# DethRaid/AndroidRenderer

Hardware: AMD Instinct MI355X
Metric: lit Mpixels/sec (deferred+GI pass) at 4K (higher is better)
Workload: dtype f32

## Files before the change

androidrenderer_amd/csrc/lighting.hip:

```cpp
#include <hip/hip_runtime.h>

#include <type_traits>

#include "../../include/sah_hip.h"
#include "fast_pixel_map.hpp"
#include "lighting_common.hpp"
#include "lighting_fast.hpp"
#include "launch.hpp"
#include "numerics.hpp"
#include "params.hpp"

namespace sah {

template <int SUN, int GI, int PPT>
__global__ void __launch_bounds__(256) k_lighting_general(const LightingArgs a, const CsmArgs csm, const LpvArgs lpv, const SkyArgs sky) {
    __shared__ float s_lut[512];
    stage_format_tables(s_lut, a.luts);
    __syncthreads();

    const uint32_t groups_per_row = a.width / PPT;
    const uint32_t gid = blockIdx.x * 256u + threadIdx.x;
    const uint32_t rows = a.row_end - a.row_begin;
    if (gid >= groups_per_row * rows) return;
    const uint32_t ry = gid / groups_per_row;
// ... 124 lines not shown
    bool neg_zero = false;
    auto put = [&](uint32_t at, float v) {
        out[at] = v;
        neg_zero = neg_zero || __float_as_uint(v) == 0x80000000u;
    };
    if (i < a.width) {
        put(i, colx_glsl_of(a, f, i));
        put(stride + i, colx_slang_of(a, f, i));
    }
    if (i < a.height) {
        put(2u * stride + i, rowy_glsl_of(a, f, i));
        put(2u * stride + row_stride + i, rowy_slang_of(a, f, i));
    }
    if (wave_any(neg_zero) && (threadIdx.x & 63u) == 0u) atomicOr(&f.state->colx_neg_zero, 1u);
}


template <int SUN, int GI, int PPT, bool SKY>
__global__ void __launch_bounds__(256, SKY ? 4 : 1) k_lighting_fast(const LightingArgs a, const CsmArgs csm, const LpvArgs lpv, const SkyArgs sky,
                                                                                 const FastArgs f) {
    uint32_t block_id = blockIdx.x;
    if (SKY) {
        if (blockIdx.x < f.sky_first) {
            const uint32_t ratio = f.sky_ratio;
            const uint32_t groups_per_row = a.width / PPT, rows = a.row_end - a.row_begin, total = groups_per_row * rows;
#pragma unroll 1
            for (uint32_t k = 0; k < ratio; k++) {
                const uint32_t gid = (blockIdx.x * ratio + k) * 256u + threadIdx.x;
                if (gid >= total) break;
                const FastPixel at = fast_pixel_of(gid, groups_per_row, rows, PPT, f.tile_rows, f.row_magic);
                const uint32_t y = a.row_begin + at.row, x0 = at.x0;
                uint32_t wz[PPT];
                load_words<PPT>(a.depth.ptr + (size_t)y * a.depth.pitch + (size_t)x0 * 4, wz);
#pragma unroll 1
                for (int i = 0; i < PPT; i++) {
                    if (__uint_as_float(wz[i]) != 0.f) continue;
                    Hn lit[4];
                    sky_frag(a, sky, x0 + (uint32_t)i, y, lit);
                    *reinterpret_cast<uint2*>(const_cast<uint8_t*>(a.lit.ptr) + (size_t)y * a.lit.pitch + (size_t)(x0 + i) * 8) = pack_lit(lit);
                }
            }
            return;
        }
        block_id = blockIdx.x - f.sky_first;
    }
    const uint32_t groups_per_row = a.width / PPT;
    const uint32_t gid = block_id * 256u + threadIdx.x;
    const uint32_t rows = a.row_end - a.row_begin;
    const bool active = gid < groups_per_row * rows;
    FastPixel at = {0u, 0u};
    if (active) at = fast_pixel_of(gid, groups_per_row, rows, PPT, f.tile_rows, f.row_magic);
    const uint32_t y = a.row_begin + at.row;
    const uint32_t x0 = at.x0;
    const bool lpv_bad = (GI == SAH_GI_LPV) ? (f.state->nonfinite != 0u) : false;
    const bool div_shared = (SUN == SAH_SHADOW_MODE_CSM || GI == SAH_GI_LPV) ? pos_div_shared_of(f) : false;

    uint32_t wc[PPT], wd[PPT], we[PPT], wz[PPT], wn[2 * PPT], wao[PPT], wm[PPT];
    float colx_g[PPT], colx_s[PPT];
    if (active) {
        load_words<PPT>(a.color.ptr + (size_t)y * a.color.pitch + (size_t)x0 * 4, wc);
        load_words<PPT>(a.data.ptr + (size_t)y * a.data.pitch + (size_t)x0 * 4, wd);
        load_words<PPT>(a.emission.ptr + (size_t)y * a.emission.pitch + (size_t)x0 * 4, we);
        load_words<PPT>(a.depth.ptr + (size_t)y * a.depth.pitch + (size_t)x0 * 4, wz);
        load_words<2 * PPT>(a.normals.ptr + (size_t)y * a.normals.pitch + (size_t)x0 * 8, wn);
        if (GI == SAH_GI_LPV && a.has_ao) load_words<PPT>(a.ao.ptr + (size_t)y * a.ao.pitch + (size_t)x0 * 4, wao);
        if (SUN == SAH_SHADOW_MODE_RT && a.has_mask) load_words<PPT>(a.shadow_mask.ptr + (size_t)y * a.shadow_mask.pitch + (size_t)x0 * 4, wm);
        if (f.colx_tab) {
            uint32_t t[PPT];
            if (SUN == SAH_SHADOW_MODE_CSM || GI == SAH_GI_LPV) {
                load_words<PPT>(reinterpret_cast<const uint8_t*>(f.colx_tab + x0), t);
#pragma unroll
                for (int i = 0; i < PPT; i++) colx_g[i] = __uint_as_float(t[i]);
            }
            if (SUN == SAH_SHADOW_MODE_RT) {
                load_words<PPT>(reinterpret_cast<const uint8_t*>(f.colx_tab + f.colx_stride + x0), t);
#pragma unroll
                for (int i = 0; i < PPT; i++) colx_s[i] = __uint_as_float(t[i]);
            }
        }
    }
    __shared__ __attribute__((aligned(16))) float s_lut[TAB_SIZE];
    stage_fast_tables<SUN == SAH_SHADOW_MODE_CSM, GI == SAH_GI_LPV>(s_lut, a, csm, f);
    __syncthreads();

    float rowy_glsl = 0.f, rowy_slang = 0.f;
    if (f.colx_tab) {
        if (SUN == SAH_SHADOW_MODE_CSM || GI == SAH_GI_LPV) rowy_glsl = f.colx_tab[2u * f.colx_stride + y];
        if (SUN == SAH_SHADOW_MODE_RT) rowy_slang = f.colx_tab[2u * f.colx_stride + f.rowy_stride + y];
    } else {
        if (SUN == SAH_SHADOW_MODE_CSM || GI == SAH_GI_LPV) rowy_glsl = rowy_glsl_of(a, f, y);
        if (SUN == SAH_SHADOW_MODE_RT) rowy_slang = rowy_slang_of(a, f, y);
    }

    uint32_t out[2 * PPT];
    uint32_t deferred_mask = 0, sky_mask = 0;
    bool emissive_wave;
    {
        uint32_t any_e = 0;
#pragma unroll
        for (int i = 0; i < PPT; i++) any_e |= we[i];
        emissive_wave = wave_any(active && (any_e & 0xffffffu) != 0u);
    }
#pragma unroll
    for (int i = 0; i < PPT; i++) {
        if (!active) break;
        Px p;
        p.color = wc[i];
        p.data = wd[i];
        p.emission = we[i];
        p.n01 = wn[2 * i];
        p.n23 = wn[2 * i + 1];
        p.depth = __uint_as_float(wz[i]);
        p.ao = (GI == SAH_GI_LPV && a.has_ao) ? __uint_as_float(wao[i]) : 1.0f;
        p.mask = (SUN == SAH_SHADOW_MODE_RT && a.has_mask) ? __uint_as_float(wm[i]) : 1.0f;
        const uint32_t x = x0 + i;
        float colx_glsl = 0.f, colx_slang = 0.f;
        if (f.colx_tab) {
            if (SUN == SAH_SHADOW_MODE_CSM || GI == SAH_GI_LPV) colx_glsl = colx_g[i];
            if (SUN == SAH_SHADOW_MODE_RT) colx_slang = colx_s[i];
        } else {
            if (SUN == SAH_SHADOW_MODE_CSM || GI == SAH_GI_LPV) colx_glsl = colx_glsl_of(a, f, x);
            if (SUN == SAH_SHADOW_MODE_RT) colx_slang = colx_slang_of(a, f, x);
        }
        const FastPixelOut r = shade_pixel_fast_sl<SUN, GI>(a, csm, lpv, f, colx_glsl, rowy_glsl, colx_slang, rowy_slang, p, s_lut, lpv_bad, emissive_wave, div_shared);
        out[2 * i] = r.lit.x;
        out[2 * i + 1] = r.lit.y;
        if (r.deferred) deferred_mask |= 1u << i;
        if (p.depth == 0.f) sky_mask |= 1u << i;
    }
    if (active) {
        uint8_t* dst = const_cast<uint8_t*>(a.lit.ptr) + (size_t)y * a.lit.pitch + (size_t)x0 * 8;
        if (SKY && sky_mask != 0u) {
#pragma unroll
            for (int i = 0; i < PPT; i++)
                if (!((sky_mask >> i) & 1u)) *reinterpret_cast<uint2*>(dst + 8 * i) = make_uint2(out[2 * i], out[2 * i + 1]);
        } else if constexpr (PPT == 1) {
            *reinterpret_cast<uint2*>(dst) = make_uint2(out[0], out[1]);
        } else {
            store_words<2 * PPT>(dst, out);
        }
    }
    const uint32_t seg = gid >> 6, lane = threadIdx.x & 63u;
    uint32_t front = 0;
    const uint32_t listed = SKY ? deferred_mask & ~sky_mask : deferred_mask;
    if (wave_any(listed != 0u)) {
        uint8_t* seg_codes = f.seg_list + (size_t)seg * f.seg_stride;
#pragma unroll
        for (int i = 0; i < PPT; i++) {
            const bool mine = (listed >> i) & 1u;
            const uint64_t m = __ballot(mine);
            if (m) {
                const uint32_t before = __builtin_amdgcn_mbcnt_hi((uint32_t)(m >> 32), __builtin_amdgcn_mbcnt_lo((uint32_t)m, 0u));
                if (mine) seg_codes[front + before] = (uint8_t)(lane * PPT + (uint32_t)i);
                front += (uint32_t)__builtin_popcountll(m);
            }
        }
    }
    if (lane == 0 && seg < f.num_segments) {
        f.seg_count[seg] = (uint16_t)front;
        if (front != 0u) f.state->deferred_hint[f.hint_slot] = 1u;
    }
    if (gid == 0u) f.state->deferred_hint[f.hint_slot ^ 1u] = 0u;
}

static hipError_t launch_lpv_pack(const LpvArgs& lpv, const FastArgs& f, hipStream_t st) {
    const uint32_t prows = (lpv.red.height + 2 * kLpvPackBorder) * (lpv.red.depth + 2 * kLpvPackBorder);
    const hipError_t me = hipMemsetAsync(&f.state->nonfinite, 0, sizeof(uint32_t), st);
    if (me != hipSuccess) return me;
    hipLaunchKernelGGL(k_lpv_pack, dim3(prows), dim3(256), 0, st, lpv.red, lpv.green, lpv.blue, const_cast<uint8_t*>(f.lpv_packed), f.pk_row_pitch,
                       f.pk_slice_pitch, f.state);
    return hipGetLastError();
}
template <int SUN, int GI>
static hipError_t launch_general_ppt(const LightingArgs& a, const CsmArgs& csm, const LpvArgs& lpv, const SkyArgs& sky, int ppt, hipStream_t st) {
    const uint32_t rows = a.row_end - a.row_begin;
    const uint64_t groups = (uint64_t)(a.width / ppt) * rows;
    if (groups == 0) return hipSuccess;
    const dim3 grid((uint32_t)((groups + 255) / 256)), block(256);
    if (ppt == 4) hipLaunchKernelGGL((k_lighting_general<SUN, GI, 4>), grid, block, 0, st, a, csm, lpv, sky);
    else if (ppt == 2) hipLaunchKernelGGL((k_lighting_general<SUN, GI, 2>), grid, block, 0, st, a, csm, lpv, sky);
    else hipLaunchKernelGGL((k_lighting_general<SUN, GI, 1>), grid, block, 0, st, a, csm, lpv, sky);
    return hipGetLastError();
}

template <int SUN, int GI>
static hipError_t launch_fast_ppt(const LightingArgs& a, const CsmArgs& csm, const LpvArgs& lpv, const SkyArgs& sky, const FastArgs& f, int ppt,
                                  hipStream_t st) {
    const uint32_t rows = a.row_end - a.row_begin;
    const uint64_t groups = (uint64_t)(a.width / ppt) * rows;
    if (groups == 0) return hipSuccess;
    if (GI == SAH_GI_LPV && f.repack) {
        const hipError_t pe = launch_lpv_pack(lpv, f, st);
        if (pe != hipSuccess) return pe;
    }
    const uint32_t blocks = (uint32_t)((groups + 255) / 256);
    const dim3 block(256);
    auto launch = [&](auto ppt_c) {
        constexpr int P = decltype(ppt_c)::value;
        if (sky.enabled) hipLaunchKernelGGL((k_lighting_fast<SUN, GI, P, true>), dim3(f.sky_first + blocks), block, 0, st, a, csm, lpv, sky, f);
        else hipLaunchKernelGGL((k_lighting_fast<SUN, GI, P, false>), dim3(blocks), block, 0, st, a, csm, lpv, sky, f);
    };
    if (ppt == 4) launch(std::integral_constant<int, 4>{});
    else if (ppt == 2) launch(std::integral_constant<int, 2>{});
    else launch(std::integral_constant<int, 1>{});
    const uint32_t fgroups = (f.num_segments + kFixupSegs - 1) / kFixupSegs;
    const dim3 fgrid(fgroups < kFixupMaxWorkgroups ? fgroups : kFixupMaxWorkgroups);
    if (ppt == 4) hipLaunchKernelGGL((k_lighting_fixup<SUN, GI, 4>), fgrid, block, 0, st, a, csm, lpv, sky, f);
// ... 44 lines not shown
```

androidrenderer_amd/csrc/lighting_common.hpp:

```cpp
#pragma once
#include <hip/hip_runtime.h>

#include "../../include/sah_hip.h"
#include "numerics.hpp"
#include "params.hpp"

namespace sah {

template <int NW> SAH_DEV void load_words(const uint8_t* p, uint32_t (&w)[NW]) {
    if constexpr (NW == 1) {
        w[0] = *reinterpret_cast<const uint32_t*>(p);
    } else if constexpr (NW == 2) {
        uint2 v = *reinterpret_cast<const uint2*>(p);
        w[0] = v.x; w[1] = v.y;
    } else if constexpr (NW == 4) {
        uint4 v = *reinterpret_cast<const uint4*>(p);
        w[0] = v.x; w[1] = v.y; w[2] = v.z; w[3] = v.w;
    } else {
        static_assert(NW == 8, "unsupported width");
        uint4 v0 = *reinterpret_cast<const uint4*>(p);
        uint4 v1 = *reinterpret_cast<const uint4*>(p + 16);
        w[0] = v0.x; w[1] = v0.y; w[2] = v0.z; w[3] = v0.w;
        w[4] = v1.x; w[5] = v1.y; w[6] = v1.z; w[7] = v1.w;
    }
}
template <int NW> SAH_DEV void store_words(uint8_t* p, const uint32_t (&w)[NW]) {
    if constexpr (NW == 2) {
        *reinterpret_cast<uint2*>(p) = make_uint2(w[0], w[1]);
    } else if constexpr (NW == 4) {
        *reinterpret_cast<uint4*>(p) = make_uint4(w[0], w[1], w[2], w[3]);
    } else {
        static_assert(NW == 8, "unsupported width");
        *reinterpret_cast<uint4*>(p) = make_uint4(w[0], w[1], w[2], w[3]);
        *reinterpret_cast<uint4*>(p + 16) = make_uint4(w[4], w[5], w[6], w[7]);
    }
}

struct Px {
    uint32_t color, data, emission, n01, n23;
    float depth, ao, mask;
};

SAH_DEV int clamp_to_int(float f) { return (int)__builtin_fminf(__builtin_fmaxf(f, -1.0e9f), 1.0e9f); }
SAH_DEV int clamp_index(float f, int hi) {
    int i, r;
    asm("v_cvt_i32_f32 %0, %1" : "=v"(i) : "v"(f));
    asm("v_med3_i32 %0, %1, 0, %2" : "=v"(r) : "v"(i), "s"(hi));
    return r;
}
SAH_DEV _Float16 hbits(uint32_t b) { return __builtin_bit_cast(_Float16, (uint16_t)b); }


struct TriSetup {
    float w[8];
    int x0, y0, z0;
    bool nan;
};
SAH_DEV TriSetup tri_setup(uint32_t W, uint32_t H, uint32_t D, float u, float v, float ww) {
    TriSetup s;
    const float px = u * (float)W - 0.5f, py = v * (float)H - 0.5f, pz = ww * (float)D - 0.5f;
    s.nan = isnan_f(px) || isnan_f(py) || isnan_f(pz);
    const float fx0 = __builtin_floorf(px), fy0 = __builtin_floorf(py), fz0 = __builtin_floorf(pz);
    const float fx = px - fx0, fy = py - fy0, fz = pz - fz0;
    const float wx0 = 1.0f - fx, wy0 = 1.0f - fy, wz0 = 1.0f - fz;
    s.x0 = clamp_to_int(fx0);
    s.y0 = clamp_to_int(fy0);
    s.z0 = clamp_to_int(fz0);
    const float wxy[4] = {wx0 * wy0, fx * wy0, wx0 * fy, fx * fy};
#pragma unroll
    for (int k = 0; k < 8; k++) s.w[k] = wxy[k & 3] * ((k >> 2) ? fz : wz0);
    return s;
}
typedef _Float16 half4_t __attribute__((ext_vector_type(4)));

SAH_DEV half4_t load_texel8_border(const VolumeArg& v, int x, int y, int z) {
    if ((unsigned)x < v.width && (unsigned)y < v.height && (unsigned)z < v.depth) {
        const uint32_t off = (uint32_t)z * v.slice_pitch + (uint32_t)y * v.row_pitch + (uint32_t)x * 8u;
        return *reinterpret_cast<const half4_t*>(v.ptr + off);
    }
    return half4_t{(_Float16)0.f, (_Float16)0.f, (_Float16)0.f, (_Float16)0.f};
}
SAH_DEV void tri_accumulate(const VolumeArg& v, const TriSetup& s, float (&out)[4]) {
    if (s.nan) {
        out[0] = out[1] = out[2] = out[3] = __builtin_nanf("");
        return;
    }
    half4_t t[8];
#pragma unroll
    for (int k = 0; k < 8; k++) t[k] = load_texel8_border(v, s.x0 + (k & 1), s.y0 + ((k >> 1) & 1), s.z0 + (k >> 2));
    out[0] = out[1] = out[2] = out[3] = 0.0f;
// ... 159 lines not shown
    s.base_color = {Hn(si.color[0]), Hn(si.color[1]), Hn(si.color[2])};
    s.normal = normalize(H3{Hn(si.normal[0]), Hn(si.normal[1]), Hn(si.normal[2])});
    s.roughness = Hn(si.rough);
    s.metalness = Hn(si.metal);
    const F3 location = worldspace_location_slang(a, (float)x, (float)y, p.depth);
    const F3 L = {Fn(a.sun_L[0]), Fn(a.sun_L[1]), Fn(a.sun_L[2])};
    const Hn ndotl = Hn(nclamp(dot(L, to_f(s.normal)), Fn(0.f), Fn(1.f)).v);
    const H3 V = to_h(normalize(location - F3{Fn(a.view_pos[0]), Fn(a.view_pos[1]), Fn(a.view_pos[2])}));
    const H3 Lh = to_h(L);
    const H3 b = brdf_sl(s, Lh, V);
    const H3 nb = ndotl * b;
    F3 radiance = to_f(nb) * F3{Fn(a.sun_color[0]), Fn(a.sun_color[1]), Fn(a.sun_color[2])};
    if (tof(ndotl) > 0.f) radiance = radiance * Fn(p.mask);
    const Fn exposure = Fn(0.00031415927f);
    add[0] = (radiance.x * exposure).v;
    add[1] = (radiance.y * exposure).v;
    add[2] = (radiance.z * exposure).v;
}

SAH_DEV void dir_to_sh(F3 d, Fn (&o)[4]) {
    const Fn c0 = Fn(0.282094792f), c1 = Fn(0.488602512f);
    o[0] = c0;
    o[1] = -c1 * d.y;
    o[2] = c1 * d.z;
    o[3] = -c1 * d.x;
}
SAH_DEV Fn dot4(const float (&t)[4], const Fn (&n)[4]) { return Fn(t[0]) * n[0] + Fn(t[1]) * n[1] + Fn(t[2]) * n[2] + Fn(t[3]) * n[3]; }

SAH_DEV void lpv_fetch(const LpvArgs& L, F4 p, const Fn (&n)[4], Fn (&out)[3]) {
    const TriSetup s = tri_setup(L.red.width, L.red.height, L.red.depth, p.x.v, p.y.v, p.z.v);
    float r[4], g[4], b[4];
    tri_accumulate(L.red, s, r);
    tri_accumulate(L.green, s, g);
    tri_accumulate(L.blue, s, b);
    out[0] = dot4(r, n);
    out[1] = dot4(g, n);
    out[2] = dot4(b, n);
}

SAH_DEV void lpv_fetch_packed(const LpvArgs& L, const uint8_t* packed, uint32_t row_pitch, uint32_t slice_pitch, float u, float v, float w,
                              const Fn (&n)[4], Fn (&out)[3]) {
    const int W = (int)L.red.width, H = (int)L.red.height, D = (int)L.red.depth;
    const float px = u * (float)W - 0.5f, py = v * (float)H - 0.5f, pz = w * (float)D - 0.5f;
    const float fx0 = __builtin_floorf(px), fy0 = __builtin_floorf(py), fz0 = __builtin_floorf(pz);
    const float fx = px - fx0, fy = py - fy0, fz = pz - fz0;
    const float gx = 1.0f - fx, gy = 1.0f - fy, gz = 1.0f - fz;
    const int b = (int)kLpvPackBorder;
    const uint32_t x0 = (uint32_t)(min(max(clamp_to_int(fx0), -b), W) + b), y0 = (uint32_t)(min(max(clamp_to_int(fy0), -b), H) + b),
                   z0 = (uint32_t)(min(max(clamp_to_int(fz0), -b), D) + b);
    const uint32_t base = z0 * slice_pitch + y0 * row_pitch + x0 * kLpvPackTexel;
    const uint32_t ro[4] = {base, base + row_pitch, base + slice_pitch, base + slice_pitch + row_pitch};
    uint32_t d[4][12];
#pragma unroll
    for (int r = 0; r < 4; r++) {
#pragma unroll
        for (int j = 0; j < 3; j++) {
            const uint4 q = *reinterpret_cast<const uint4*>(packed + ro[r] + 16u * (uint32_t)j);
            d[r][4 * j] = q.x;
            d[r][4 * j + 1] = q.y;
            d[r][4 * j + 2] = q.z;
            d[r][4 * j + 3] = q.w;
        }
    }
    const float wxy[4] = {gx * gy, fx * gy, gx * fy, fx * fy};
    float wt[8];
#pragma unroll
    for (int k = 0; k < 8; k++) wt[k] = wxy[k & 3] * ((k >> 2) ? fz : gz);
#pragma unroll
    for (int c = 0; c < 3; c++) {
        float a[4] = {0.f, 0.f, 0.f, 0.f};
#pragma unroll
        for (int k = 0; k < 8; k++) {
            const int r = k >> 1, xs = k & 1;
            const uint32_t lo = d[r][xs * 6 + c * 2], hi = d[r][xs * 6 + c * 2 + 1];
            a[0] = fma_mix_lo(wt[k], lo, a[0]);
            a[1] = fma_mix_hi(wt[k], lo, a[1]);
            a[2] = fma_mix_lo(wt[k], hi, a[2]);
            a[3] = fma_mix_hi(wt[k], hi, a[3]);
        }
        out[c] = dot4(a, n);
    }
}

SAH_DEV void gi_lpv_frag(const LightingArgs& a, const LpvArgs& L, uint32_t x, uint32_t y, const Px& p, const SurfIn& si, Fn (&out)[4]) {
    Surface<Fn> s;
    s.base_color = {Fn(si.color[0]), Fn(si.color[1]), Fn(si.color[2])};
    s.normal = normalize(F3{Fn(si.normal[0]), Fn(si.normal[1]), Fn(si.normal[2])});
    s.roughness = Fn(si.rough);
    s.metalness = Fn(si.metal);
    const F3 vs = viewspace_position_glsl(a, x, y, p.depth);
    const F4 ws = mul44(a.inv_view, F4{vs.x, vs.y, vs.z, Fn(1.0f)});
    const F3 V = normalize(F3{ws.x, ws.y, ws.z} - F3{Fn(a.view_pos[0]), Fn(a.view_pos[1]), Fn(a.view_pos[2])});

    uint32_t selected = 0;
    for (int i = (int)L.num_cascades - 1; i >= 0; i--) {
        const F4 cp = mul44(L.world_to_cascade[i], ws);
        if (cp.x.v > 0.f && cp.y.v > 0.f && cp.z.v > 0.f && cp.x.v < 1.f && cp.y.v < 1.f && cp.z.v < 1.f) selected = (uint32_t)i;
    }
    F3 lpv_normal = -s.normal;
    lpv_normal.x = lpv_normal.x * Fn(-1.0f);
    Fn nc[4];
    dir_to_sh(lpv_normal, nc);

    Fn indirect[3];
    {
        const F4 pos = {ws.x + s.normal.x, ws.y + s.normal.y, ws.z + s.normal.z, ws.w + Fn(0.f)};
        F4 cp = mul44(L.world_to_cascade[selected], pos);
        cp.x = cp.x + Fn((float)selected);
        cp.x = cp.x / Fn(L.num_cascades_f);
        lpv_fetch(L, cp, nc, indirect);
    }
    const F3 I = -V;
    const F3 refl = I - s.normal * (Fn(2.0f) * dot(s.normal, I));
    Fn spec[3] = {Fn(0.f), Fn(0.f), Fn(0.f)};
    if (selected == 0) {
        const F4 cp = mul44(L.world_to_cascade[0], ws);
        Fn rc[4];
        dir_to_sh(refl, rc);
        lpv_fetch(L, cp, rc, spec);
        const F3 loc = F3{ws.x, ws.y, ws.z} + refl * Fn(1.0f);
        const F4 cp1 = mul44(L.world_to_cascade[0], F4{loc.x, loc.y, loc.z, Fn(1.f)});
        Fn more[3];
        lpv_fetch(L, cp1, rc, more);
#pragma unroll
        for (int i = 0; i < 3; i++) spec[i] = (spec[i] + more[i]) / Fn(2.0f);
    }
    const F3 diffuse_factor = Fd(s, s.normal, s.normal);
    const F3 fr = Fr(s, s.normal, refl);
    const F3 specular_factor = {fr.x * Fn(0.f), fr.y * Fn(0.f), fr.z * Fn(0.f)};
    const Fn ao = Fn(p.ao);
    F3 total = {indirect[0] * diffuse_factor.x * ao + spec[0] * specular_factor.x,
                indirect[1] * diffuse_factor.y * ao + spec[1] * specular_factor.y,
                indirect[2] * diffuse_factor.z * ao + spec[2] * specular_factor.z};
    if (any_nan(total)) total = F3(Fn(0.f));
    const Fn exposure = Fn(L.exposure);
    out[0] = total.x * exposure;
    out[1] = total.y * exposure;
    out[2] = total.z * exposure;
    out[3] = Fn(1.0f);
}

SAH_DEV Fn cr_acos(Fn x) { return Fn((float)acos((double)x.v)); }
SAH_DEV Fn cr_atan(Fn x) { return Fn((float)atan((double)x.v)); }
SAH_DEV Fn cr_exp(Fn x) { return Fn((float)exp((double)x.v)); }
SAH_DEV Fn fsign(Fn x) { return Fn(x.v > 0.f ? 1.0f : (x.v < 0.f ? -1.0f : 0.0f)); }

SAH_DEV Fn ray_intersect_sphere(F3 ro, F3 rd, Fn rad) {
    const Fn b = dot(ro, rd);
    const Fn c = dot(ro, ro) - rad * rad;
    if (c.v > 0.0f && b.v > 0.0f) return Fn(-1.0f);
    const Fn discr = b * b - c;
    if (discr.v < 0.0f) return Fn(-1.0f);
    if (discr.v > (b * b).v) return (-b + nsqrt(discr));
    return -b - nsqrt(discr);
}

SAH_DEV F3 sky_color(const SkyArgs& k, F3 rayDir) {
    const Fn sky_pi = Fn(3.14159265358f);
    const F3 sunDir = {Fn(k.sun_dir[0]), Fn(k.sun_dir[1]), Fn(k.sun_dir[2])};
    const F3 up = {Fn(0.0f) / Fn(k.height), Fn(k.up_y), Fn(0.0f) / Fn(k.height)};
    const F3 view_pos = {Fn(0.f), Fn(k.view_pos_y), Fn(0.f)};

    const Fn altitudeAngle = Fn(k.horizon_angle) - cr_acos(dot(rayDir, up));
    Fn azimuthAngle;
    if (__builtin_fabsf(altitudeAngle.v) > k.azimuth_limit) {
        azimuthAngle = Fn(0.0f);
// ... 121 lines not shown
```

androidrenderer_amd/csrc/lighting_fast.hpp:

```cpp
#pragma once
#include "lighting_common.hpp"

namespace sah {

SAH_DEV bool finite_f(float x) { return __builtin_fabsf(x) < __builtin_inff(); }

enum : uint32_t { TAB_CSM = 512, TAB_LPV = 512 + 48, TAB_VIEW = 512 + 48 + 32, TAB_SIZE = 512 + 48 + 32 + 12 };

SAH_DEV void stage_format_tables(float* s_lut, const float* luts) {
    s_lut[threadIdx.x] = luts[threadIdx.x];
    s_lut[threadIdx.x + 256] = luts[threadIdx.x + 256];
}
template <bool CSM, bool LPV>
SAH_DEV void stage_fast_tables(float* s_lut, const LightingArgs& a, const CsmArgs& csm, const FastArgs& f) {
    stage_format_tables(s_lut, a.luts);
    if (CSM && threadIdx.x < 48) {
        const uint32_t c = threadIdx.x / 12u, j = threadIdx.x % 12u;
        s_lut[TAB_CSM + threadIdx.x] = csm.biased[c][(j & 3u) * 4u + (j >> 2)];
    }
    if (LPV && threadIdx.x >= 64 && threadIdx.x < 96) {
        const uint32_t t = threadIdx.x - 64u, c = t >> 3, j = t & 7u;
        s_lut[TAB_LPV + t] = (j & 3u) == 3u ? 0.f : (j < 4u ? f.lpv_s[c][j] : f.lpv_t[c][j - 4u]);
    }
    if (threadIdx.x >= 128 && threadIdx.x < 140) {
        const uint32_t t = threadIdx.x - 128u;
        s_lut[TAB_VIEW + t] = a.inv_view[(t & 3u) * 4u + (t >> 2)];
    }
}

SAH_DEV float colx_glsl_of(const LightingArgs& a, const FastArgs& f, uint32_t x) {
    const Fn tx = (Fn((float)x + 0.5f) + Fn(0.5f)) / Fn(a.res[0]);
    return (Fn(f.p0) * (tx * Fn(2.0f) - Fn(1.0f)) + Fn(f.p12)).v;
}
SAH_DEV float colx_slang_of(const LightingArgs& a, const FastArgs& f, uint32_t x) {
    const Fn tx = (Fn((float)x) + Fn(0.5f)) / Fn(a.res[0]);
    return (Fn(f.p0) * (tx * Fn(2.0f) - Fn(1.0f)) + Fn(f.p12)).v;
}
SAH_DEV float rowy_glsl_of(const LightingArgs& a, const FastArgs& f, uint32_t y) {
    const Fn ty = (Fn((float)y + 0.5f) + Fn(0.5f)) / Fn(a.res[1]);
    return (Fn(f.p5) * (ty * Fn(2.0f) - Fn(1.0f)) + Fn(f.p13)).v;
}
SAH_DEV float rowy_slang_of(const LightingArgs& a, const FastArgs& f, uint32_t y) {
    const Fn ty = (Fn((float)y) + Fn(0.5f)) / Fn(a.res[1]);
    return (Fn(f.p5) * (ty * Fn(2.0f) - Fn(1.0f)) + Fn(f.p13)).v;
}

SAH_DEV bool pos_div_shared_of(const FastArgs& f) { return f.pos_div_nr != 0u || (f.pos_div_shared != 0u && f.state->colx_neg_zero == 0u); }

struct FastPixelOut {
    uint2 lit;
    bool deferred;
};

struct FastGeom {
    F3 N, ws, V;
    Fn vsz;
};
SAH_DEV FastGeom fast_geometry(const LightingArgs& a, const FastArgs& f, float colx_glsl, float rowy_glsl, float D, const SurfIn& si, float dn,
                               const float* tab, bool div_shared, bool& ok) {
    FastGeom g;
    const Fn inv = Fn(rcp_nr(sqrt_nr(dn)));
    g.N = F3{Fn(si.normal[0]) * inv, Fn(si.normal[1]) * inv, Fn(si.normal[2]) * inv};
    const Fn vw = Fn(f.p11) * Fn(D) + Fn(f.p15);
    const Fn vzn = Fn(f.p10) * Fn(D) + Fn(f.p14);
    Fn vx, vy;
    if (div_shared) {
        const float aw = __builtin_fabsf(vw.v);
        ok = ok && aw >= kDivLo && aw <= kDivHi;
        const float y0 = __builtin_amdgcn_rcpf(vw.v);
        const float y1 = __builtin_fmaf(__builtin_fmaf(-vw.v, y0, 1.0f), y0, y0);
        auto quot = [&](float num) {
            const float q0 = num * y1;
            const float q1 = __builtin_fmaf(__builtin_fmaf(-vw.v, q0, num), y1, q0);
            return Fn(__builtin_fmaf(__builtin_fmaf(-vw.v, q1, num), y1, q1));
        };
        vx = quot(colx_glsl);
        vy = quot(rowy_glsl);
        g.vsz = quot(vzn.v);
    } else {
        vx = Fn(colx_glsl) / vw;
        vy = Fn(rowy_glsl) / vw;
        g.vsz = vzn / vw;
    }
    const float4 mx = *reinterpret_cast<const float4*>(tab + TAB_VIEW), my = *reinterpret_cast<const float4*>(tab + TAB_VIEW + 4u),
                 mz = *reinterpret_cast<const float4*>(tab + TAB_VIEW + 8u);
    g.ws.x = Fn(mx.x) * vx + Fn(mx.y) * vy + Fn(mx.z) * g.vsz + Fn(mx.w);
    g.ws.y = Fn(my.x) * vx + Fn(my.y) * vy + Fn(my.z) * g.vsz + Fn(my.w);
    g.ws.z = Fn(mz.x) * vx + Fn(mz.y) * vy + Fn(mz.z) * g.vsz + Fn(mz.w);
    const F3 d = g.ws - F3{Fn(a.view_pos[0]), Fn(a.view_pos[1]), Fn(a.view_pos[2])};
    const Fn d2 = dot(d, d);
    ok = ok && d2.v >= 0x1p-80f && d2.v <= 0x1p+80f;
    g.V = d * Fn(rcp_nr(sqrt_nr(d2.v)));
    return g;
}

SAH_DEV void fast_csm_sun(const LightingArgs& a, const CsmArgs& csm, const float* tab, const F3& N, const F3& ws, const Fn vsz, const F3& V, const F3& L,
                          const Surface<Fn>& s, const SurfIn& si, lanemask act, bool& ok, Fn (&sc)[3]) {
    const Fn ndotl_sun = nclamp(dot(N, L), Fn(0.f), Fn(1.f));
    sc[0] = sc[1] = sc[2] = Fn(0.f);
    const lanemask lit_m = lanes(ndotl_sun.v > 0.f) & act;
    if (lit_m) {
        uint32_t cascade = 0;
#pragma unroll
        for (uint32_t i = 0; i < 4; i++) cascade = (vsz.v < csm.splits[i]) ? i + 1u : cascade;
        const uint32_t cc = cascade > 3u ? 3u : cascade;
        const Fn bias_num = Fn(0.0005f) * Fn(sqrt_nr0((Fn(1.0f) - ndotl_sun * ndotl_sun).v));
        const Fn bias = Fn(div_nr(bias_num.v, ndotl_sun.v));
        ok = ok && !(ndotl_sun.v > 0.f && ndotl_sun.v < kDivLo);
        const float4 rx = *reinterpret_cast<const float4*>(tab + TAB_CSM + cc * 12u);
        const float4 ry = *reinterpret_cast<const float4*>(tab + TAB_CSM + cc * 12u + 4u);
        const float4 rz = *reinterpret_cast<const float4*>(tab + TAB_CSM + cc * 12u + 8u);
        const Fn spx = Fn(rx.x) * ws.x + Fn(rx.y) * ws.y + Fn(rx.z) * ws.z + Fn(rx.w);
        const Fn spy = Fn(ry.x) * ws.x + Fn(ry.y) * ws.y + Fn(ry.z) * ws.z + Fn(ry.w);
        const Fn spz = Fn(rz.x) * ws.x + Fn(rz.y) * ws.y + Fn(rz.z) * ws.z + Fn(rz.w);
        const float sp_mn = __builtin_fminf(__builtin_fminf(spx.v, spy.v), spz.v), sp_mx = __builtin_fmaxf(__builtin_fmaxf(spx.v, spy.v), spz.v);
        const bool sp_inside = !(sp_mn < 0.f || sp_mx > 1.f);
        float pcf_ref = (spz - bias).v;
        pcf_ref = pcf_ref < 0.f ? 0.f : (pcf_ref > 1.f ? 1.f : pcf_ref);
        const VolumeArg& sm = csm.shadowmap;
        const float px = spx.v * (float)sm.width - 0.5f, py = spy.v * (float)sm.height - 0.5f;
        const float fx0 = __builtin_floorf(px), fy0 = __builtin_floorf(py);
        const float pcf_fx = px - fx0, pcf_fy = py - fy0;
        const int wm1 = (int)sm.width - 1, hm1 = (int)sm.height - 1;
        const uint32_t xa = (uint32_t)clamp_index(fx0, wm1) * 2u, xb = (uint32_t)clamp_index(fx0 + 1.0f, wm1) * 2u;
        const uint32_t ra = (uint32_t)clamp_index(fy0, hm1) * sm.row_pitch, rb = (uint32_t)clamp_index(fy0 + 1.0f, hm1) * sm.row_pitch;
        const uint32_t lo = cc * sm.slice_pitch;
        const uint32_t pcf_off[4] = {lo + ra + xa, lo + ra + xb, lo + rb + xa, lo + rb + xb};
        float dtap[4];
        uint16_t raw[4];
#pragma unroll
        for (int k = 0; k < 4; k++) raw[k] = *reinterpret_cast<const uint16_t*>(sm.ptr + pcf_off[k]);
#pragma unroll
        for (int k = 0; k < 4; k++) {
            const float v = (float)raw[k];
            const float q = v * csm.d16_recip;
            dtap[k] = __builtin_fmaf(__builtin_fmaf(-q, 65535.0f, v), csm.d16_recip, q);
        }
        const float wx0 = 1.0f - pcf_fx, wy0 = 1.0f - pcf_fy;
        float pcf = __builtin_fmaf(wx0 * wy0, (pcf_ref < dtap[0]) ? 1.0f : 0.0f, 0.0f);
        pcf = __builtin_fmaf(pcf_fx * wy0, (pcf_ref < dtap[1]) ? 1.0f : 0.0f, pcf);
        pcf = __builtin_fmaf(wx0 * pcf_fy, (pcf_ref < dtap[2]) ? 1.0f : 0.0f, pcf);
        pcf = __builtin_fmaf(pcf_fx * pcf_fy, (pcf_ref < dtap[3]) ? 1.0f : 0.0f, pcf);
        float shadow = sp_inside ? pcf : 1.0f;
        shadow = cascade > 3u ? 0.0f : shadow;
        shadow = ndotl_sun.v > 0.f ? shadow : 1.0f;
        if (lit_m & lanes(shadow != 0.0f)) {
            bool brdf_out_of_domain;
            const F3 b = brdf_fast(s, L, V, brdf_out_of_domain);
            const F3 direct = ndotl_sun * b * F3{Fn(a.sun_color[0]), Fn(a.sun_color[1]), Fn(a.sun_color[2])} * Fn(shadow);
            const float nan_probe = (direct.x + direct.y + direct.z).v;
            ok = ok && !brdf_out_of_domain && nan_probe == nan_probe;
            const Fn exposure = Fn(0.00031415927f);
            sc[0] = direct.x * exposure;
            sc[1] = direct.y * exposure;
            sc[2] = direct.z * exposure;
        }
    }
}

SAH_DEV void fast_lpv_overlay(const LpvArgs& lpv, const FastArgs& f, const float* tab, F3 N, F3 ws, const SurfIn& si, float ao_px, lanemask act, bool& ok,
                              float (&add)[3]) {
    lanemask out_m = 0;
    auto inside = [&](uint32_t i) {
        const float4 cs_ = *reinterpret_cast<const float4*>(tab + TAB_LPV + i * 8u);
        const float4 ct_ = *reinterpret_cast<const float4*>(tab + TAB_LPV + i * 8u + 4u);
        const Fn cx = Fn(cs_.x) * ws.x + Fn(ct_.x);
        const Fn cy = Fn(cs_.y) * ws.y + Fn(ct_.y);
        const Fn cz = Fn(cs_.z) * ws.z + Fn(ct_.z);
        const float mn = __builtin_fminf(__builtin_fminf(cx.v, cy.v), cz.v), mxv = __builtin_fmaxf(__builtin_fmaxf(cx.v, cy.v), cz.v);
        out_m = lanes(!(mn > 0.f)) | lanes(!(mxv < 1.f));
        return mn > 0.f && mxv < 1.f;
    };
    uint32_t selected = 0;
    const bool in0 = inside(0u);
    if (out_m & act) {
#pragma unroll
        for (int i = 3; i >= 1; i--) {
            if (i < (int)lpv.num_cascades) selected = inside((uint32_t)i) ? (uint32_t)i : selected;
        }
        selected = in0 ? 0u : selected;
    }
    F3 lpv_normal = -N;
    lpv_normal.x = lpv_normal.x * Fn(-1.0f);
    Fn nc[4];
    dir_to_sh(lpv_normal, nc);
    const float4 cs = *reinterpret_cast<const float4*>(tab + TAB_LPV + selected * 8u);
    const float4 ct = *reinterpret_cast<const float4*>(tab + TAB_LPV + selected * 8u + 4u);
    Fn cpx = Fn(cs.x) * (ws.x + N.x) + Fn(ct.x);
    const Fn cpy = Fn(cs.y) * (ws.y + N.y) + Fn(ct.y);
    const Fn cpz = Fn(cs.z) * (ws.z + N.z) + Fn(ct.z);
    cpx = cpx + Fn((float)selected);
    cpx = f.ncasc_pow2 ? cpx * Fn(f.inv_ncasc) : cpx / Fn(lpv.num_cascades_f);
    Fn indirect[3];
    lpv_fetch_packed(lpv, f.lpv_packed, f.pk_row_pitch, f.pk_slice_pitch, cpx.v, cpy.v, cpz.v, nc, indirect);
    const Fn dielectric_f0 = Fn(0.04f);
    const F3 base_color = {Fn(si.color[0]), Fn(si.color[1]), Fn(si.color[2])};
    const F3 diffuse_color = base_color * (Fn(1.0f) - dielectric_f0) * (Fn(1.0f) - Fn(si.metal));
    const Fn inv_pi = (Fn(1.0f) * Fn(1.0f)) * (Fn(1.0f) / Fn(3.1415927f));
    const F3 diffuse_factor = diffuse_color * inv_pi;
    const Fn ao = Fn(ao_px);
    const F3 total = {indirect[0] * diffuse_factor.x * ao, indirect[1] * diffuse_factor.y * ao, indirect[2] * diffuse_factor.z * ao};
    const float nan_probe = (total.x + total.y + total.z).v;
    ok = ok && nan_probe == nan_probe;
    const Fn exposure = Fn(lpv.exposure);
    add[0] = (total.x * exposure).v;
    add[1] = (total.y * exposure).v;
    add[2] = (total.z * exposure).v;
}

template <int SUN, int GI>
SAH_DEV FastPixelOut shade_pixel_fast_sl(const LightingArgs& a, const CsmArgs& csm, const LpvArgs& lpv, const FastArgs& f, float colx_glsl,
                                         float rowy_glsl, float colx_slang, float rowy_slang, const Px& p, const float* tab,
                                         bool lpv_has_nonfinite, bool emissive_wave, bool div_shared) {
    const float* lut = tab;
    const float D = p.depth;
    const bool sky_px = D == 0.f;
    const uint32_t rough_byte = (p.data >> 8) & 0xffu;
    const SurfIn si = unpack_surface(p, lut);
    const float dn = (si.normal[0] * si.normal[0] + si.normal[1] * si.normal[1]) + si.normal[2] * si.normal[2];
    bool ok = finite_f(D) && dn > 0.f && finite_f(dn);
    if (GI == SAH_GI_LPV) ok = ok && rough_byte != 0u && !lpv_has_nonfinite;

    Hn lit[4] = {Hn::lit(0.f), Hn::lit(0.f), Hn::lit(0.f), Hn::lit(0.f)};

    F3 N, ws, V;
    Fn vsz;
    if (SUN == SAH_SHADOW_MODE_CSM || GI == SAH_GI_LPV) {
        const FastGeom g = fast_geometry(a, f, colx_glsl, rowy_glsl, D, si, dn, tab, div_shared, ok);
        N = g.N;
        ws = g.ws;
        V = g.V;
        vsz = g.vsz;
    }

    Surface<Fn> s;
    s.base_color = {Fn(si.color[0]), Fn(si.color[1]), Fn(si.color[2])};
    s.normal = N;
    s.roughness = Fn(si.rough);
    s.metalness = Fn(si.metal);
    const lanemask act = lanes(ok && !sky_px);

    const F3 L = {Fn(a.sun_L[0]), Fn(a.sun_L[1]), Fn(a.sun_L[2])};
    Fn nc[4];
    float lpv_u = 0.f, lpv_v = 0.f, lpv_w = 0.f;
    if constexpr (GI == SAH_GI_LPV) {
        lanemask out_m = 0;
        auto inside = [&](uint32_t i) {
            const float4 cs_ = *reinterpret_cast<const float4*>(tab + TAB_LPV + i * 8u);
            const float4 ct_ = *reinterpret_cast<const float4*>(tab + TAB_LPV + i * 8u + 4u);
            const Fn cx = Fn(cs_.x) * ws.x + Fn(ct_.x);
            const Fn cy = Fn(cs_.y) * ws.y + Fn(ct_.y);
            const Fn cz = Fn(cs_.z) * ws.z + Fn(ct_.z);
            const float mn = __builtin_fminf(__builtin_fminf(cx.v, cy.v), cz.v), mxv = __builtin_fmaxf(__builtin_fmaxf(cx.v, cy.v), cz.v);
            out_m = lanes(!(mn > 0.f)) | lanes(!(mxv < 1.f));
            return mn > 0.f && mxv < 1.f;
        };
        uint32_t selected = 0;
        const bool in0 = inside(0u);
        if (out_m & act) {
#pragma unroll
            for (int i = 3; i >= 1; i--) {
                if (i < (int)lpv.num_cascades) selected = inside((uint32_t)i) ? (uint32_t)i : selected;
            }
            selected = in0 ? 0u : selected;
        }
        F3 lpv_normal = -N;
        lpv_normal.x = lpv_normal.x * Fn(-1.0f);
        dir_to_sh(lpv_normal, nc);
        const float4 cs = *reinterpret_cast<const float4*>(tab + TAB_LPV + selected * 8u);
        const float4 ct = *reinterpret_cast<const float4*>(tab + TAB_LPV + selected * 8u + 4u);
        Fn cpx = Fn(cs.x) * (ws.x + N.x) + Fn(ct.x);
        const Fn cpy = Fn(cs.y) * (ws.y + N.y) + Fn(ct.y);
        const Fn cpz = Fn(cs.z) * (ws.z + N.z) + Fn(ct.z);
        cpx = cpx + Fn((float)selected);
        cpx = f.ncasc_pow2 ? cpx * Fn(f.inv_ncasc) : cpx / Fn(lpv.num_cascades_f);
        lpv_u = cpx.v;
        lpv_v = cpy.v;
        lpv_w = cpz.v;
    }

    if constexpr (SUN == SAH_SHADOW_MODE_CSM) {
        Fn sc[3];
        fast_csm_sun(a, csm, tab, N, ws, vsz, V, L, s, si, act, ok, sc);
        const bool quirk = (a.flags & SAH_LIGHTING_QUIRK_SUN_BLEND) != 0;
        float x1[3];
#pragma unroll
        for (int i = 0; i < 3; i++) x1[i] = quirk ? (sc[i] * sc[i]).v : (Fn(0.f) + sc[i]).v;
#pragma unroll
        for (int i = 0; i < 3; i++) lit[i] = Hn(x1[i]);
        lit[3] = quirk ? Hn::lit(0.0f) : Hn::lit(1.0f);
    }

    if constexpr (GI == SAH_GI_LPV) {
        Fn indirect[3];
        lpv_fetch_packed(lpv, f.lpv_packed, f.pk_row_pitch, f.pk_slice_pitch, lpv_u, lpv_v, lpv_w, nc, indirect);
        const Fn dielectric_f0 = Fn(0.04f);
        const F3 diffuse_color = s.base_color * (Fn(1.0f) - dielectric_f0) * (Fn(1.0f) - s.metalness);
        const Fn inv_pi = (Fn(1.0f) * Fn(1.0f)) * (Fn(1.0f) / Fn(3.1415927f));
        const F3 diffuse_factor = diffuse_color * inv_pi;
        const Fn ao = Fn(p.ao);
        const F3 total = {indirect[0] * diffuse_factor.x * ao, indirect[1] * diffuse_factor.y * ao, indirect[2] * diffuse_factor.z * ao};
        const float nan_probe = (total.x + total.y + total.z).v;
        ok = ok && nan_probe == nan_probe;
        const Fn exposure = Fn(lpv.exposure);
        lit[0] = Hn(tof(lit[0]) + (total.x * exposure).v);
        lit[1] = Hn(tof(lit[1]) + (total.y * exposure).v);
        lit[2] = Hn(tof(lit[2]) + (total.z * exposure).v);
        lit[3] = lit[3] + Hn::lit(1.0f);
    }

    float er = 0.f, eg = 0.f, eb = 0.f;
    if (emissive_wave) {
        const Fn e = Fn(3.1415927f);
        er = (Fn(lut[p.emission & 0xffu]) * e).v;
        eg = (Fn(lut[(p.emission >> 8) & 0xffu]) * e).v;
        eb = (Fn(lut[(p.emission >> 16) & 0xffu]) * e).v;
        lit[0] = Hn(tof(lit[0]) + er);
        lit[1] = Hn(tof(lit[1]) + eg);
        lit[2] = Hn(tof(lit[2]) + eb);
    } else {
#pragma unroll
        for (int i = 0; i < 3; i++) lit[i] = lit[i] + Hn::lit(0.f);
    }
    lit[3] = lit[3] + Hn::lit(1.0f);

    if constexpr (SUN == SAH_SHADOW_MODE_RT) {
        Surface<Hn> sh;
        sh.base_color = {Hn(si.color[0]), Hn(si.color[1]), Hn(si.color[2])};
        sh.normal = normalize(H3{Hn(si.normal[0]), Hn(si.normal[1]), Hn(si.normal[2])});
        sh.roughness = Hn(si.rough);
        sh.metalness = Hn(si.metal);
        const Fn vw = Fn(f.p11) * Fn(D) + Fn(f.p15);
        const Fn vx = Fn(colx_slang) / vw, vy = Fn(rowy_slang) / vw, vz = (Fn(f.p10) * Fn(D) + Fn(f.p14)) / vw;
        const Fn vww = vw / vw;
        const float* m = a.inv_view;
        F3 loc;
        loc.x = Fn(m[0]) * vx + Fn(m[4]) * vy + Fn(m[8]) * vz + Fn(m[12]) * vww;
        loc.y = Fn(m[1]) * vx + Fn(m[5]) * vy + Fn(m[9]) * vz + Fn(m[13]) * vww;
        loc.z = Fn(m[2]) * vx + Fn(m[6]) * vy + Fn(m[10]) * vz + Fn(m[14]) * vww;
        const Hn ndotl = Hn(nclamp(dot(L, to_f(sh.normal)), Fn(0.f), Fn(1.f)).v);
        const H3 Vh = to_h(normalize(loc - F3{Fn(a.view_pos[0]), Fn(a.view_pos[1]), Fn(a.view_pos[2])}));
        const H3 Lh = to_h(L);
        const H3 b = brdf_sl(sh, Lh, Vh);
        const H3 nb = ndotl * b;
        F3 radiance = to_f(nb) * F3{Fn(a.sun_color[0]), Fn(a.sun_color[1]), Fn(a.sun_color[2])};
        const F3 masked = radiance * Fn(p.mask);
        const bool lit_side = tof(ndotl) > 0.f;
        radiance = {lit_side ? masked.x : radiance.x, lit_side ? masked.y : radiance.y, lit_side ? masked.z : radiance.z};
        const Fn exposure = Fn(0.00031415927f);
        lit[0] = Hn(tof(lit[0]) + (radiance.x * exposure).v);
        lit[1] = Hn(tof(lit[1]) + (radiance.y * exposure).v);
        lit[2] = Hn(tof(lit[2]) + (radiance.z * exposure).v);
    }

    FastPixelOut o;
    Hn sky_lit[4] = {Hn(er), Hn(eg), Hn(eb), Hn::lit(1.0f)};
    const uint2 surf = pack_lit(lit), bare = pack_lit(sky_lit);
    o.lit.x = sky_px ? bare.x : surf.x;
    o.lit.y = sky_px ? bare.y : surf.y;
    o.deferred = sky_px ? (f.sky_enabled != 0u) : !ok;
    return o;
}

}
```

Baseline: 56230.

## Stage per-wave 4x4x4 LPV box in LDS and trilinear-fetch from it

```diff
diff --git a/androidrenderer_amd/csrc/lighting.hip b/androidrenderer_amd/csrc/lighting.hip
--- a/androidrenderer_amd/csrc/lighting.hip
+++ b/androidrenderer_amd/csrc/lighting.hip
@@ -230,6 +230,13 @@
     __shared__ __attribute__((aligned(16))) float s_lut[TAB_SIZE];
     stage_fast_tables<SUN == SAH_SHADOW_MODE_CSM, GI == SAH_GI_LPV>(s_lut, a, csm, f);
     __syncthreads();
+    LpvBox box;
+    box.lds = nullptr;
+    box.valid = false;
+    if constexpr (GI == SAH_GI_LPV) {
+        __shared__ __attribute__((aligned(16))) uint8_t s_box[4 * kLpvBoxBytes];
+        box.lds = s_box + (uint32_t)__builtin_amdgcn_readfirstlane((int)(threadIdx.x >> 6)) * kLpvBoxBytes;
+    }
 
     float rowy_glsl = 0.f, rowy_slang = 0.f;
     if (f.colx_tab) {
@@ -270,7 +277,8 @@
             if (SUN == SAH_SHADOW_MODE_CSM || GI == SAH_GI_LPV) colx_glsl = colx_glsl_of(a, f, x);
             if (SUN == SAH_SHADOW_MODE_RT) colx_slang = colx_slang_of(a, f, x);
         }
-        const FastPixelOut r = shade_pixel_fast_sl<SUN, GI>(a, csm, lpv, f, colx_glsl, rowy_glsl, colx_slang, rowy_slang, p, s_lut, lpv_bad, emissive_wave, div_shared);
+        const FastPixelOut r = shade_pixel_fast_sl<SUN, GI>(a, csm, lpv, f, colx_glsl, rowy_glsl, colx_slang, rowy_slang, p, s_lut, lpv_bad, emissive_wave, div_shared, box, i == 0,
+                                                                   lpv_box_centre_lane(PPT));
         out[2 * i] = r.lit.x;
         out[2 * i + 1] = r.lit.y;
         if (r.deferred) deferred_mask |= 1u << i;
diff --git a/androidrenderer_amd/csrc/lighting_common.hpp b/androidrenderer_amd/csrc/lighting_common.hpp
--- a/androidrenderer_amd/csrc/lighting_common.hpp
+++ b/androidrenderer_amd/csrc/lighting_common.hpp
@@ -2,10 +2,13 @@
 #include <hip/hip_runtime.h>
 
 #include "../../include/sah_hip.h"
+#include "lpv_box.hpp"
 #include "numerics.hpp"
 #include "params.hpp"
 
 namespace sah {
+
+static_assert(kLpvBoxSrcTexel == kLpvPackTexel && kLpvBoxPad == kLpvPackBorder, "lpv_box.hpp restates the gather copy's texel and border");
 
 template <int NW> SAH_DEV void load_words(const uint8_t* p, uint32_t (&w)[NW]) {
     if constexpr (NW == 1) {
@@ -331,6 +334,41 @@
     }
 }
 
+SAH_DEV void lpv_packed_base(const LpvArgs& L, float u, float v, float w, uint32_t (&base)[3]) {
+    const int W = (int)L.red.width, H = (int)L.red.height, D = (int)L.red.depth;
+    const float px = u * (float)W - 0.5f, py = v * (float)H - 0.5f, pz = w * (float)D - 0.5f;
+    const float fx0 = __builtin_floorf(px), fy0 = __builtin_floorf(py), fz0 = __builtin_floorf(pz);
+    const int b = (int)kLpvPackBorder;
+    base[0] = (uint32_t)(min(max(clamp_to_int(fx0), -b), W) + b);
+    base[1] = (uint32_t)(min(max(clamp_to_int(fy0), -b), H) + b);
+    base[2] = (uint32_t)(min(max(clamp_to_int(fz0), -b), D) + b);
+}
+
+SAH_DEV void lpv_fetch_box(const LpvArgs& L, const uint8_t* box_px, float u, float v, float w, const Fn (&n)[4], Fn (&out)[3]) {
+    const int W = (int)L.red.width, H = (int)L.red.height, D = (int)L.red.depth;
+    const float px = u * (float)W - 0.5f, py = v * (float)H - 0.5f, pz = w * (float)D - 0.5f;
+    const float fx0 = __builtin_floorf(px), fy0 = __builtin_floorf(py), fz0 = __builtin_floorf(pz);
+    const float fx = px - fx0, fy = py - fy0, fz = pz - fz0;
+    const float gx = 1.0f - fx, gy = 1.0f - fy, gz = 1.0f - fz;
+    const float wxy[4] = {gx * gy, fx * gy, gx * fy, fx * fy};
+    float wt[8];
+#pragma unroll
+    for (int k = 0; k < 8; k++) wt[k] = wxy[k & 3] * ((k >> 2) ? fz : gz);
+#pragma unroll
+    for (int c = 0; c < 3; c++) {
+        float a[4] = {0.f, 0.f, 0.f, 0.f};
+#pragma unroll
+        for (int k = 0; k < 8; k++) {
+            const float4 t = *reinterpret_cast<const float4*>(box_px + lpv_box_lds_row((uint32_t)k >> 1) + (uint32_t)(k & 1) * kLpvBoxTexel + 16u * (uint32_t)c);
+            a[0] = __builtin_fmaf(wt[k], t.x, a[0]);
+            a[1] = __builtin_fmaf(wt[k], t.y, a[1]);
+            a[2] = __builtin_fmaf(wt[k], t.z, a[2]);
+            a[3] = __builtin_fmaf(wt[k], t.w, a[3]);
+        }
+        out[c] = dot4(a, n);
+    }
+}
+
 SAH_DEV void gi_lpv_frag(const LightingArgs& a, const LpvArgs& L, uint32_t x, uint32_t y, const Px& p, const SurfIn& si, Fn (&out)[4]) {
     Surface<Fn> s;
     s.base_color = {Fn(si.color[0]), Fn(si.color[1]), Fn(si.color[2])};
diff --git a/androidrenderer_amd/csrc/lighting_fast.hpp b/androidrenderer_amd/csrc/lighting_fast.hpp
--- a/androidrenderer_amd/csrc/lighting_fast.hpp
+++ b/androidrenderer_amd/csrc/lighting_fast.hpp
@@ -51,6 +51,34 @@
     uint2 lit;
     bool deferred;
 };
+
+struct LpvBox {
+    uint8_t* lds;
+    bool valid;
+    uint32_t o[3];
+    uint4 q[2];
+};
+SAH_DEV void lpv_box_request(LpvBox& box, const FastArgs& f) {
+    const uint32_t lane = threadIdx.x & 63u;
+    const uint32_t c[2] = {lane, 64u + (lane & 31u)};
+#pragma unroll
+    for (int i = 0; i < 2; i++)
+        box.q[i] = *reinterpret_cast<const uint4*>(f.lpv_packed + lpv_box_chunk_src(c[i], box.o[0], box.o[1], box.o[2], f.pk_row_pitch, f.pk_slice_pitch));
+}
+SAH_DEV void lpv_box_write(const LpvBox& box) {
+    const uint32_t lane = threadIdx.x & 63u;
+    const uint32_t c[2] = {lane, 64u + (lane & 31u)};
+#pragma unroll
+    for (int i = 0; i < 2; i++) {
+        const uint4 q = box.q[i];
+        float4* dst = reinterpret_cast<float4*>(box.lds + lpv_box_chunk_dst(c[i]));
+        dst[0] = make_float4(h2f((uint16_t)q.x), h2f((uint16_t)(q.x >> 16)), h2f((uint16_t)q.y), h2f((uint16_t)(q.y >> 16)));
+        dst[1] = make_float4(h2f((uint16_t)q.z), h2f((uint16_t)(q.z >> 16)), h2f((uint16_t)q.w), h2f((uint16_t)(q.w >> 16)));
+    }
+    __builtin_amdgcn_fence(__ATOMIC_RELEASE, "wavefront");
+    __builtin_amdgcn_wave_barrier();
+    __builtin_amdgcn_fence(__ATOMIC_ACQUIRE, "wavefront");
+}
 
 struct FastGeom {
     F3 N, ws, V;
@@ -211,7 +239,8 @@
 template <int SUN, int GI>
 SAH_DEV FastPixelOut shade_pixel_fast_sl(const LightingArgs& a, const CsmArgs& csm, const LpvArgs& lpv, const FastArgs& f, float colx_glsl,
                                          float rowy_glsl, float colx_slang, float rowy_slang, const Px& p, const float* tab,
-                                         bool lpv_has_nonfinite, bool emissive_wave, bool div_shared) {
+                                         bool lpv_has_nonfinite, bool emissive_wave, bool div_shared, LpvBox& box, bool first_slot,
+                                         uint32_t centre_lane) {
     const float* lut = tab;
     const float D = p.depth;
     const bool sky_px = D == 0.f;
@@ -243,6 +272,8 @@
     const F3 L = {Fn(a.sun_L[0]), Fn(a.sun_L[1]), Fn(a.sun_L[2])};
     Fn nc[4];
     float lpv_u = 0.f, lpv_v = 0.f, lpv_w = 0.f;
+    bool box_tap = false;
+    const uint8_t* box_px = nullptr;
     if constexpr (GI == SAH_GI_LPV) {
         lanemask out_m = 0;
         auto inside = [&](uint32_t i) {
@@ -277,6 +308,26 @@
         lpv_u = cpx.v;
         lpv_v = cpy.v;
         lpv_w = cpz.v;
+        uint32_t lb[3];
+        lpv_packed_base(lpv, lpv_u, lpv_v, lpv_w, lb);
+        const uint32_t size[3] = {lpv.red.width, lpv.red.height, lpv.red.depth};
+        if (first_slot) {
+            box.valid = false;
+            box.o[0] = box.o[1] = box.o[2] = 0u;
+            if (act) {
+                const uint32_t ref = lpv_box_reference_lane(act, centre_lane);
+#pragma unroll
+                for (int k = 0; k < 3; k++) box.o[k] = lpv_box_origin((uint32_t)__builtin_amdgcn_readlane((int)lb[k], (int)ref), size[k]);
+            }
+        }
+        const uint32_t dx = lpv_box_delta(lb[0], box.o[0]), dy = lpv_box_delta(lb[1], box.o[1]), dz = lpv_box_delta(lb[2], box.o[2]);
+        const lanemask unserved = lanes(max(max(dx, dy), dz) > kLpvBoxEdge - 2u) & act;
+        if (first_slot && act != 0ull && unserved == 0ull && lanes(true) == ~0ull) {
+            box.valid = true;
+            lpv_box_request(box, f);
+        }
+        box_tap = box.valid && unserved == 0ull;
+        box_px = box.lds + lpv_box_lds_base(lpv_box_clamp_delta(dx), lpv_box_clamp_delta(dy), lpv_box_clamp_delta(dz));
     }
 
     if constexpr (SUN == SAH_SHADOW_MODE_CSM) {
@@ -293,7 +344,9 @@
 
     if constexpr (GI == SAH_GI_LPV) {
         Fn indirect[3];
-        lpv_fetch_packed(lpv, f.lpv_packed, f.pk_row_pitch, f.pk_slice_pitch, lpv_u, lpv_v, lpv_w, nc, indirect);
+        if (first_slot && box.valid) lpv_box_write(box);
+        if (box_tap) lpv_fetch_box(lpv, box_px, lpv_u, lpv_v, lpv_w, nc, indirect);
+        else lpv_fetch_packed(lpv, f.lpv_packed, f.pk_row_pitch, f.pk_slice_pitch, lpv_u, lpv_v, lpv_w, nc, indirect);
         const Fn dielectric_f0 = Fn(0.04f);
         const F3 diffuse_color = s.base_color * (Fn(1.0f) - dielectric_f0) * (Fn(1.0f) - s.metalness);
         const Fn inv_pi = (Fn(1.0f) * Fn(1.0f)) * (Fn(1.0f) / Fn(3.1415927f));
diff --git a/androidrenderer_amd/csrc/lpv_box.hpp b/androidrenderer_amd/csrc/lpv_box.hpp
--- /dev/null
+++ b/androidrenderer_amd/csrc/lpv_box.hpp
@@ -0,0 +1,56 @@
+#pragma once
+#include <stdint.h>
+
+#if defined(__HIPCC__) || defined(__CUDACC__)
+#define SAH_LPV_BOX_FN __host__ __device__ inline
+#else
+#define SAH_LPV_BOX_FN inline
+#endif
+
+namespace sah {
+
+constexpr uint32_t kLpvBoxEdge = 4;
+constexpr uint32_t kLpvBoxSrcTexel = 24, kLpvBoxPad = 2;
+constexpr uint32_t kLpvBoxTexel = 2 * kLpvBoxSrcTexel;
+constexpr uint32_t kLpvBoxRow = kLpvBoxEdge * kLpvBoxTexel;
+constexpr uint32_t kLpvBoxSlab = kLpvBoxEdge * kLpvBoxRow + 16;
+constexpr uint32_t kLpvBoxBytes = kLpvBoxEdge * kLpvBoxSlab;
+constexpr uint32_t kLpvBoxSrcRow = kLpvBoxEdge * kLpvBoxSrcTexel;
+constexpr uint32_t kLpvBoxChunksPerRow = kLpvBoxSrcRow / 16;
+constexpr uint32_t kLpvBoxChunks = kLpvBoxEdge * kLpvBoxEdge * kLpvBoxChunksPerRow;
+
+SAH_LPV_BOX_FN uint32_t lpv_box_padded(uint32_t size) { return size + 2u * kLpvBoxPad; }
+
+SAH_LPV_BOX_FN uint32_t lpv_box_origin(uint32_t r, uint32_t size) {
+    const uint32_t hi = lpv_box_padded(size) - kLpvBoxEdge;
+    const uint32_t lo = r == 0u ? 0u : r - 1u;
+    return lo < hi ? lo : hi;
+}
+
+SAH_LPV_BOX_FN uint32_t lpv_box_delta(uint32_t base, uint32_t o) { return base - o; }
+SAH_LPV_BOX_FN bool lpv_box_served(uint32_t dx, uint32_t dy, uint32_t dz) {
+    return dx <= kLpvBoxEdge - 2u && dy <= kLpvBoxEdge - 2u && dz <= kLpvBoxEdge - 2u;
+}
+SAH_LPV_BOX_FN uint32_t lpv_box_clamp_delta(uint32_t d) { return d < kLpvBoxEdge - 2u ? d : kLpvBoxEdge - 2u; }
+
+SAH_LPV_BOX_FN uint32_t lpv_box_lds_base(uint32_t dx, uint32_t dy, uint32_t dz) {
+    return dz * kLpvBoxSlab + dy * kLpvBoxRow + dx * kLpvBoxTexel;
+}
+SAH_LPV_BOX_FN uint32_t lpv_box_lds_row(uint32_t k) { return (k >> 1) * kLpvBoxSlab + (k & 1u) * kLpvBoxRow; }
+
+SAH_LPV_BOX_FN uint32_t lpv_box_chunk_src(uint32_t c, uint32_t ox, uint32_t oy, uint32_t oz, uint32_t row_pitch, uint32_t slice_pitch) {
+    const uint32_t row = c / kLpvBoxChunksPerRow, j = c - row * kLpvBoxChunksPerRow;
+    return (oz + row / kLpvBoxEdge) * slice_pitch + (oy + row % kLpvBoxEdge) * row_pitch + ox * kLpvBoxSrcTexel + 16u * j;
+}
+SAH_LPV_BOX_FN uint32_t lpv_box_chunk_dst(uint32_t c) {
+    const uint32_t row = c / kLpvBoxChunksPerRow, j = c - row * kLpvBoxChunksPerRow;
+    return (row / kLpvBoxEdge) * kLpvBoxSlab + (row % kLpvBoxEdge) * kLpvBoxRow + 32u * j;
+}
+
+SAH_LPV_BOX_FN uint32_t lpv_box_centre_lane(uint32_t ppt) { return (ppt / 2u) * (64u / ppt) + 32u / ppt; }
+SAH_LPV_BOX_FN uint32_t lpv_box_reference_lane(uint64_t act, uint32_t centre) {
+    const uint64_t behind = act & (~0ull << centre);
+    return behind ? (uint32_t)__builtin_ctzll(behind) : 63u - (uint32_t)__builtin_clzll(act);
+}
+
+}
```

Result: faster. 60380, median of 6 (+7.4%).
